# zju3dv/Diffuman4D

Measured on NVIDIA H100. Metric: unet_window_denoise_steps_per_sec, higher is better.
Workload: dtype bf16

## Files before the change

diffuman4d_b200/build.py:

```python
from __future__ import annotations

import concurrent.futures as cf
import os
import subprocess
import sys

HERE = os.path.dirname(os.path.abspath(__file__))
CSRC = os.path.join(HERE, "csrc")
OBJ = os.path.join(HERE, "_obj")
LIB = os.path.join(HERE, "libd4d.so")
SOURCES = ["tmap.cu", "gemm_wgmma.cu", "attention_wgmma.cu", "norm.cu", "elementwise.cu", "unet.cu", "d4d_api.cu"]
NVCC = os.environ.get("NVCC", "/usr/local/cuda/bin/nvcc")
FLAGS = ["-std=c++17", "-O3", "-gencode", "arch=compute_90a,code=sm_90a", "-lineinfo", "-Xcompiler", "-fPIC",
         "-diag-suppress", "177"]


def _deps_mtime() -> float:
    t = 0.0
    for root in (CSRC, os.path.join(HERE, "..", "include")):
        for f in os.listdir(root):
            if f.endswith((".h", ".cuh")):
                t = max(t, os.path.getmtime(os.path.join(root, f)))
    return t


def _compile(src: str, force: bool, hdr_t: float) -> str:
    obj = os.path.join(OBJ, src.replace(".cu", ".o"))
    s = os.path.join(CSRC, src)
    if not force and os.path.exists(obj) and os.path.getmtime(obj) >= max(os.path.getmtime(s), hdr_t):
        return obj
    cmd = [NVCC, *FLAGS, "-I", CSRC, "-c", s, "-o", obj]
    r = subprocess.run(cmd, capture_output=True, text=True)
    if r.returncode != 0:
        raise RuntimeError(f"nvcc failed for {src}:\n{r.stdout}\n{r.stderr}")
    return obj


def _link(lib: str, objs, force: bool) -> bool:
    need_link = force or not os.path.exists(lib) or any(os.path.getmtime(o) > os.path.getmtime(lib) for o in objs)
    if need_link:
        cmd = [NVCC, "-shared", "-o", lib, *objs, "-cudart", "static", "-gencode", "arch=compute_90a,code=sm_90a",
               "-Xlinker", "--exclude-libs,ALL"]
        r = subprocess.run(cmd, capture_output=True, text=True)
        if r.returncode != 0:
            raise RuntimeError(f"link failed:\n{r.stdout}\n{r.stderr}")
    return need_link


def build(force: bool = False, verbose: bool = True) -> str:
    os.makedirs(OBJ, exist_ok=True)
    hdr_t = _deps_mtime()
    with cf.ThreadPoolExecutor(max_workers=min(8, os.cpu_count() or 4)) as ex:
        objs = list(ex.map(lambda s: _compile(s, force, hdr_t), SOURCES))
    linked = _link(LIB, objs, force)
    if verbose:
        print(f"[d4d] {'built' if linked else 'up to date'}: {LIB}")
    return LIB


if __name__ == "__main__":
    build(force="--force" in sys.argv)
```

diffuman4d_b200/csrc/attention_wgmma.cu:

```cuda
#include <math.h>

#include "kernels.h"
#include "wgmma.cuh"

namespace d4d {

namespace {

constexpr int BLOCK_Q = 128;
constexpr int BLOCK_KV = 64;
constexpr int ATT_THREADS = 288;
constexpr int QBOX_BYTES = BLOCK_Q * 64 * 2;
constexpr int KVBOX_BYTES = BLOCK_KV * 64 * 2;

template <int NB>
struct AttCfg {
  static constexpr int D = 64 * NB;
  static constexpr int STAGES = NB == 3 ? 3 : 4;
  static constexpr int Q_BYTES = QBOX_BYTES * NB;
  static constexpr int STAGE_BYTES = 2 * KVBOX_BYTES * NB;
  static constexpr int SMEM_BYTES = 1024 + Q_BYTES + STAGES * STAGE_BYTES + 256;
  static constexpr int MIN_BLOCKS = NB == 1 ? 2 : 1;
};

struct AttKernelArgs {
  int seq_q, seq_kv, heads, n_kv_tiles;
  float scale_log2;
  bf16* out;
  int ld_out;
};

__device__ __forceinline__ float ex2_approx(float x) {
  float y;
  asm("ex2.approx.ftz.f32 %0, %1;" : "=f"(y) : "f"(x));
  return y;
}

template <int NB>
__global__ void __launch_bounds__(ATT_THREADS, AttCfg<NB>::MIN_BLOCKS)
attn_wgmma_kernel(const __grid_constant__ CUtensorMap tmap_q, const __grid_constant__ CUtensorMap tmap_k,
                  const __grid_constant__ CUtensorMap tmap_v, const AttKernelArgs a) {
  using C = AttCfg<NB>;
  extern __shared__ uint8_t smem_raw[];
  uint8_t* smem = reinterpret_cast<uint8_t*>((reinterpret_cast<uintptr_t>(smem_raw) + 1023) & ~uintptr_t(1023));
  uint8_t* sQ = smem;
  uint8_t* ring = smem + C::Q_BYTES;
  uint64_t* kv_full = reinterpret_cast<uint64_t*>(ring + C::STAGES * C::STAGE_BYTES);
  uint64_t* kv_empty = kv_full + C::STAGES;
  uint64_t* q_full = kv_empty + C::STAGES;

  const int warp = __shfl_sync(0xffffffffu, threadIdx.x >> 5, 0);
  const int lane = threadIdx.x & 31;
  const int q_tile = blockIdx.x;
  const int bh = blockIdx.y;
  const int b = bh / a.heads;
  const int hd = bh - b * a.heads;
  const int q_row0 = b * a.seq_q;
  const int kv_row0 = b * a.seq_kv;
  const int col0 = hd * C::D;
  const int n_tiles = a.n_kv_tiles;

  if (threadIdx.x == 0) {
    for (int i = 0; i < C::STAGES; ++i) {
      mbar_init(&kv_full[i], 1);
      mbar_init(&kv_empty[i], 2);
    }
    mbar_init(q_full, 1);
    fence_mbar_init();
  }
  __syncthreads();
  pdl_wait();
  pdl_launch_dependents();

  if (warp == 8) {
    if (lane == 0) {
      tma_prefetch_desc(&tmap_q);
      tma_prefetch_desc(&tmap_k);
      tma_prefetch_desc(&tmap_v);
      mbar_expect_tx(q_full, C::Q_BYTES);
#pragma unroll
      for (int nb = 0; nb < NB; ++nb)
        tma_load_2d(sQ + nb * QBOX_BYTES, &tmap_q, q_full, col0 + nb * 64, q_row0 + q_tile * BLOCK_Q);
      int stage = 0;
      uint32_t phase = 0;
      for (int j = 0; j < n_tiles; ++j) {
        mbar_wait(&kv_empty[stage], phase ^ 1);
        uint8_t* dst = ring + stage * C::STAGE_BYTES;
        mbar_expect_tx(&kv_full[stage], C::STAGE_BYTES);
#pragma unroll
        for (int nb = 0; nb < NB; ++nb) {
          tma_load_2d(dst + nb * KVBOX_BYTES, &tmap_k, &kv_full[stage], col0 + nb * 64, kv_row0 + j * BLOCK_KV);
          tma_load_2d(dst + (NB + nb) * KVBOX_BYTES, &tmap_v, &kv_full[stage], col0 + nb * 64, kv_row0 + j * BLOCK_KV);
        }
        if (++stage == C::STAGES) { stage = 0; phase ^= 1; }
      }
    }
    return;
  }

  const int wg = warp >> 2;
  const bool wg_leader = (threadIdx.x & 127) == 0;
  const int c_base = 2 * (lane & 3);
  const uint32_t q_addr = smem_u32(sQ) + wg * 64 * 128;
  const uint32_t ring_u32 = smem_u32(ring);

  float o[NB][32];
#pragma unroll
  for (int nb = 0; nb < NB; ++nb)
#pragma unroll
    for (int i = 0; i < 32; ++i) o[nb][i] = 0.f;
  float m_run[2] = {-INFINITY, -INFINITY};
  float l_run[2] = {0.f, 0.f};
  mbar_wait(q_full, 0);

  int stage = 0;
  uint32_t phase = 0;
  for (int j = 0; j < n_tiles; ++j) {
    mbar_wait(&kv_full[stage], phase);
    const uint32_t kv = ring_u32 + stage * C::STAGE_BYTES;
    float s[32];
    wgmma_fence();
#pragma unroll
    for (int nb = 0; nb < NB; ++nb) {
      const uint64_t qd = make_wgmma_desc(q_addr + nb * QBOX_BYTES, 16, 1024);
      const uint64_t kd = make_wgmma_desc(kv + nb * KVBOX_BYTES, 16, 1024);
#pragma unroll
      for (int k = 0; k < 4; ++k) wgmma_ss_n64(s, qd + 2 * k, kd + 2 * k, (nb | k) != 0 ? 1 : 0);
    }
    wgmma_commit();
    wgmma_wait<0>();
    wgmma_fence_regs(s);

    const int valid = a.seq_kv - j * BLOCK_KV;
    if (valid < BLOCK_KV) {
#pragma unroll
      for (int i = 0; i < 32; ++i)
        if (8 * (i >> 2) + c_base + (i & 1) >= valid) s[i] = -INFINITY;
    }
    float corr[2];
#pragma unroll
    for (int h = 0; h < 2; ++h) {
      float mx = -INFINITY;
#pragma unroll
      for (int jj = 0; jj < 8; ++jj) mx = fmaxf(mx, fmaxf(s[4 * jj + 2 * h], s[4 * jj + 2 * h + 1]));
      mx = fmaxf(mx, __shfl_xor_sync(0xffffffffu, mx, 1));
      mx = fmaxf(mx, __shfl_xor_sync(0xffffffffu, mx, 2));
      const float m_new = fmaxf(m_run[h], mx * a.scale_log2);
      corr[h] = ex2_approx(m_run[h] - m_new);
      m_run[h] = m_new;
      float sum = 0.f;
#pragma unroll
      for (int jj = 0; jj < 8; ++jj) {
#pragma unroll
        for (int e = 0; e < 2; ++e) {
          const float p = ex2_approx(fmaf(s[4 * jj + 2 * h + e], a.scale_log2, -m_new));
          s[4 * jj + 2 * h + e] = p;
          sum += p;
        }
      }
      l_run[h] = l_run[h] * corr[h] + sum;
    }
#pragma unroll
    for (int nb = 0; nb < NB; ++nb)
#pragma unroll
      for (int i = 0; i < 32; ++i) o[nb][i] *= corr[(i >> 1) & 1];

    uint32_t pf[4][4];
#pragma unroll
    for (int kk = 0; kk < 4; ++kk) {
      pf[kk][0] = pack_bf16x2(s[8 * kk + 0], s[8 * kk + 1]);
      pf[kk][1] = pack_bf16x2(s[8 * kk + 2], s[8 * kk + 3]);
      pf[kk][2] = pack_bf16x2(s[8 * kk + 4], s[8 * kk + 5]);
      pf[kk][3] = pack_bf16x2(s[8 * kk + 6], s[8 * kk + 7]);
    }
    wgmma_fence();
#pragma unroll
    for (int nb = 0; nb < NB; ++nb) {
      const uint64_t vd = make_wgmma_desc(kv + (NB + nb) * KVBOX_BYTES, KVBOX_BYTES, 1024);
#pragma unroll
      for (int kk = 0; kk < 4; ++kk) wgmma_rs_n64_bmn(o[nb], pf[kk], vd + (2048 >> 4) * kk);
    }
    wgmma_commit();
    wgmma_wait<0>();
#pragma unroll
    for (int nb = 0; nb < NB; ++nb) wgmma_fence_regs(o[nb]);
    if (wg_leader) mbar_arrive(&kv_empty[stage]);
    if (++stage == C::STAGES) { stage = 0; phase ^= 1; }
  }

  const int r_base = q_tile * BLOCK_Q + wg * 64 + (warp & 3) * 16 + (lane >> 2);
#pragma unroll
  for (int h = 0; h < 2; ++h) {
    float l = l_run[h];
    l += __shfl_xor_sync(0xffffffffu, l, 1);
    l += __shfl_xor_sync(0xffffffffu, l, 2);
    const float inv_l = 1.f / l;
    const int qrow = r_base + 8 * h;
    if (qrow >= a.seq_q) continue;
    bf16* orow = a.out + static_cast<size_t>(q_row0 + qrow) * a.ld_out + col0;
#pragma unroll
    for (int nb = 0; nb < NB; ++nb)
#pragma unroll
      for (int jj = 0; jj < 8; ++jj)
        *reinterpret_cast<uint32_t*>(orow + nb * 64 + 8 * jj + c_base) =
            pack_bf16x2(o[nb][4 * jj + 2 * h] * inv_l, o[nb][4 * jj + 2 * h + 1] * inv_l);
  }
}

template <int NB>
int launch_attn(const AttnLaunch& L, cudaStream_t stream) {
  using C = AttCfg<NB>;
  static PerDeviceOnce attr_once;
  if (int rc = ensure_dyn_smem(attn_wgmma_kernel<NB>, C::SMEM_BYTES, attr_once)) return rc;
  AttKernelArgs a;
  a.seq_q = L.d.seq;
  a.seq_kv = L.d.seq_kv > 0 ? L.d.seq_kv : L.d.seq;
  a.heads = L.d.heads;
  a.n_kv_tiles = (a.seq_kv + BLOCK_KV - 1) / BLOCK_KV;
  a.scale_log2 = L.d.scale * 1.4426950408889634f;
  a.out = L.d.out;
  a.ld_out = L.d.ld_out;
  dim3 grid(L.grid_x, L.grid_y);
  D4D_CUDA_OK(launch_pdl(attn_wgmma_kernel<NB>, grid, dim3(ATT_THREADS), C::SMEM_BYTES, stream, L.tmap_q, L.tmap_k, L.tmap_v, a));
  D4D_CUDA_OK(cudaGetLastError());
  return 0;
}

}

int attn_prepare(const AttnDesc& d, AttnLaunch* L) {
  D4D_REQUIRE(d.head_dim == 64 || d.head_dim == 128 || d.head_dim == 192,
              "attention head_dim (after padding) must be 64, 128 or 192");
  D4D_REQUIRE(d.batch > 0 && d.seq > 0 && d.heads > 0 && d.seq_kv >= 0, "empty attention problem");
  D4D_REQUIRE(d.ld_qkv % 8 == 0 && d.ld_out % 8 == 0 && d.ld_kv % 8 == 0, "leading dimensions must be multiples of 8");
  D4D_REQUIRE(d.scale > 0.f, "softmax scale must be positive");
  L->d = d;
  L->variant = d.head_dim / 64;
  const int seq_kv = d.seq_kv > 0 ? d.seq_kv : d.seq;
  const int ld_kv = d.ld_kv > 0 ? d.ld_kv : d.ld_qkv;
  const uint64_t q_tokens = static_cast<uint64_t>(d.batch) * d.seq;
  const uint64_t kv_tokens = static_cast<uint64_t>(d.batch) * seq_kv;
  const uint64_t width = static_cast<uint64_t>(d.heads) * d.head_dim;
  if (int rc = make_tmap_2d(&L->tmap_q, d.q, q_tokens, width, d.ld_qkv, 64, BLOCK_Q, 128)) return rc;
  if (int rc = make_tmap_2d(&L->tmap_k, d.k, kv_tokens, width, ld_kv, 64, BLOCK_KV, 128)) return rc;
  if (int rc = make_tmap_2d(&L->tmap_v, d.v, kv_tokens, width, ld_kv, 64, BLOCK_KV, 128)) return rc;
  L->grid_x = (d.seq + BLOCK_Q - 1) / BLOCK_Q;
  L->grid_y = d.batch * d.heads;
  D4D_REQUIRE(L->grid_y <= 65535, "batch*heads exceeds grid.y limit");
  return 0;
}

int attn_run(const AttnLaunch& L, cudaStream_t stream) {
  switch (L.variant) {
    case 1: return launch_attn<1>(L, stream);
    case 2: return launch_attn<2>(L, stream);
    case 3: return launch_attn<3>(L, stream);
  }
  set_error("attention: unsupported head_dim variant");
  return 1;
}

double attn_flops(const AttnDesc& d) {
  const double skv = d.seq_kv > 0 ? d.seq_kv : d.seq;
  return 4.0 * d.batch * d.heads * static_cast<double>(d.seq) * skv * d.head_dim;
}

}
```

diffuman4d_b200/csrc/wgmma.cuh:

```cuda
#pragma once
#include <stdint.h>

namespace d4d {

__device__ __forceinline__ void wgmma_fence() { asm volatile("wgmma.fence.sync.aligned;" ::: "memory"); }
__device__ __forceinline__ void wgmma_commit() { asm volatile("wgmma.commit_group.sync.aligned;" ::: "memory"); }
template <int N> __device__ __forceinline__ void wgmma_wait() {
  asm volatile("wgmma.wait_group.sync.aligned %0;" ::"n"(N) : "memory");
}
template <int R> __device__ __forceinline__ void wgmma_fence_regs(float (&d)[R]) {
#pragma unroll
  for (int i = 0; i < R; ++i) asm volatile("" : "+f"(d[i])::"memory");
}

__device__ __forceinline__ uint64_t make_wgmma_desc(uint32_t saddr, uint32_t lbo_bytes, uint32_t sbo_bytes) {
  uint64_t d = 0;
  d |= static_cast<uint64_t>((saddr >> 4) & 0x3FFFu);
  d |= static_cast<uint64_t>((lbo_bytes >> 4) & 0x3FFFu) << 16;
  d |= static_cast<uint64_t>((sbo_bytes >> 4) & 0x3FFFu) << 32;
  d |= 1ull << 62;
  return d;
}


__device__ __forceinline__ void wgmma_ss_n64(float (&d)[32], uint64_t a_desc, uint64_t b_desc, int scale_d) {
  asm volatile(
      "{\n\t.reg .pred p;\n\t"
      "setp.ne.b32 p, %34, 0;\n\t"
      "wgmma.mma_async.sync.aligned.m64n64k16.f32.bf16.bf16 {%0, %1, %2, %3, %4, %5, %6, %7, %8, %9, %10, %11, %12, %13, %14, %15, %16, %17, %18, %19, %20, %21, %22, %23, %24, %25, %26, %27, %28, %29, %30, %31}, %32, %33, p, 1, 1, 0, 0;\n\t}\n"
      : "+f"(d[0]), "+f"(d[1]), "+f"(d[2]), "+f"(d[3]), "+f"(d[4]), "+f"(d[5]), "+f"(d[6]), "+f"(d[7]), "+f"(d[8]), "+f"(d[9]), "+f"(d[10]), "+f"(d[11]), "+f"(d[12]), "+f"(d[13]), "+f"(d[14]), "+f"(d[15]), "+f"(d[16]), "+f"(d[17]), "+f"(d[18]), "+f"(d[19]), "+f"(d[20]), "+f"(d[21]), "+f"(d[22]), "+f"(d[23]), "+f"(d[24]), "+f"(d[25]), "+f"(d[26]), "+f"(d[27]), "+f"(d[28]), "+f"(d[29]), "+f"(d[30]), "+f"(d[31])
      : "l"(a_desc), "l"(b_desc), "r"(scale_d));
}

__device__ __forceinline__ void wgmma_ss_n128(float (&d)[64], uint64_t a_desc, uint64_t b_desc, int scale_d) {
  asm volatile(
      "{\n\t.reg .pred p;\n\t"
      "setp.ne.b32 p, %66, 0;\n\t"
      "wgmma.mma_async.sync.aligned.m64n128k16.f32.bf16.bf16 {%0, %1, %2, %3, %4, %5, %6, %7, %8, %9, %10, %11, %12, %13, %14, %15, %16, %17, %18, %19, %20, %21, %22, %23, %24, %25, %26, %27, %28, %29, %30, %31, %32, %33, %34, %35, %36, %37, %38, %39, %40, %41, %42, %43, %44, %45, %46, %47, %48, %49, %50, %51, %52, %53, %54, %55, %56, %57, %58, %59, %60, %61, %62, %63}, %64, %65, p, 1, 1, 0, 0;\n\t}\n"
      : "+f"(d[0]), "+f"(d[1]), "+f"(d[2]), "+f"(d[3]), "+f"(d[4]), "+f"(d[5]), "+f"(d[6]), "+f"(d[7]), "+f"(d[8]), "+f"(d[9]), "+f"(d[10]), "+f"(d[11]), "+f"(d[12]), "+f"(d[13]), "+f"(d[14]), "+f"(d[15]), "+f"(d[16]), "+f"(d[17]), "+f"(d[18]), "+f"(d[19]), "+f"(d[20]), "+f"(d[21]), "+f"(d[22]), "+f"(d[23]), "+f"(d[24]), "+f"(d[25]), "+f"(d[26]), "+f"(d[27]), "+f"(d[28]), "+f"(d[29]), "+f"(d[30]), "+f"(d[31]), "+f"(d[32]), "+f"(d[33]), "+f"(d[34]), "+f"(d[35]), "+f"(d[36]), "+f"(d[37]), "+f"(d[38]), "+f"(d[39]), "+f"(d[40]), "+f"(d[41]), "+f"(d[42]), "+f"(d[43]), "+f"(d[44]), "+f"(d[45]), "+f"(d[46]), "+f"(d[47]), "+f"(d[48]), "+f"(d[49]), "+f"(d[50]), "+f"(d[51]), "+f"(d[52]), "+f"(d[53]), "+f"(d[54]), "+f"(d[55]), "+f"(d[56]), "+f"(d[57]), "+f"(d[58]), "+f"(d[59]), "+f"(d[60]), "+f"(d[61]), "+f"(d[62]), "+f"(d[63])
      : "l"(a_desc), "l"(b_desc), "r"(scale_d));
}

__device__ __forceinline__ void wgmma_ss_n160(float (&d)[80], uint64_t a_desc, uint64_t b_desc, int scale_d) {
  asm volatile(
      "{\n\t.reg .pred p;\n\t"
      "setp.ne.b32 p, %82, 0;\n\t"
      "wgmma.mma_async.sync.aligned.m64n160k16.f32.bf16.bf16 {%0, %1, %2, %3, %4, %5, %6, %7, %8, %9, %10, %11, %12, %13, %14, %15, %16, %17, %18, %19, %20, %21, %22, %23, %24, %25, %26, %27, %28, %29, %30, %31, %32, %33, %34, %35, %36, %37, %38, %39, %40, %41, %42, %43, %44, %45, %46, %47, %48, %49, %50, %51, %52, %53, %54, %55, %56, %57, %58, %59, %60, %61, %62, %63, %64, %65, %66, %67, %68, %69, %70, %71, %72, %73, %74, %75, %76, %77, %78, %79}, %80, %81, p, 1, 1, 0, 0;\n\t}\n"
      : "+f"(d[0]), "+f"(d[1]), "+f"(d[2]), "+f"(d[3]), "+f"(d[4]), "+f"(d[5]), "+f"(d[6]), "+f"(d[7]), "+f"(d[8]), "+f"(d[9]), "+f"(d[10]), "+f"(d[11]), "+f"(d[12]), "+f"(d[13]), "+f"(d[14]), "+f"(d[15]), "+f"(d[16]), "+f"(d[17]), "+f"(d[18]), "+f"(d[19]), "+f"(d[20]), "+f"(d[21]), "+f"(d[22]), "+f"(d[23]), "+f"(d[24]), "+f"(d[25]), "+f"(d[26]), "+f"(d[27]), "+f"(d[28]), "+f"(d[29]), "+f"(d[30]), "+f"(d[31]), "+f"(d[32]), "+f"(d[33]), "+f"(d[34]), "+f"(d[35]), "+f"(d[36]), "+f"(d[37]), "+f"(d[38]), "+f"(d[39]), "+f"(d[40]), "+f"(d[41]), "+f"(d[42]), "+f"(d[43]), "+f"(d[44]), "+f"(d[45]), "+f"(d[46]), "+f"(d[47]), "+f"(d[48]), "+f"(d[49]), "+f"(d[50]), "+f"(d[51]), "+f"(d[52]), "+f"(d[53]), "+f"(d[54]), "+f"(d[55]), "+f"(d[56]), "+f"(d[57]), "+f"(d[58]), "+f"(d[59]), "+f"(d[60]), "+f"(d[61]), "+f"(d[62]), "+f"(d[63]), "+f"(d[64]), "+f"(d[65]), "+f"(d[66]), "+f"(d[67]), "+f"(d[68]), "+f"(d[69]), "+f"(d[70]), "+f"(d[71]), "+f"(d[72]), "+f"(d[73]), "+f"(d[74]), "+f"(d[75]), "+f"(d[76]), "+f"(d[77]), "+f"(d[78]), "+f"(d[79])
      : "l"(a_desc), "l"(b_desc), "r"(scale_d));
}

__device__ __forceinline__ void wgmma_ss_n192(float (&d)[96], uint64_t a_desc, uint64_t b_desc, int scale_d) {
  asm volatile(
      "{\n\t.reg .pred p;\n\t"
      "setp.ne.b32 p, %98, 0;\n\t"
      "wgmma.mma_async.sync.aligned.m64n192k16.f32.bf16.bf16 {%0, %1, %2, %3, %4, %5, %6, %7, %8, %9, %10, %11, %12, %13, %14, %15, %16, %17, %18, %19, %20, %21, %22, %23, %24, %25, %26, %27, %28, %29, %30, %31, %32, %33, %34, %35, %36, %37, %38, %39, %40, %41, %42, %43, %44, %45, %46, %47, %48, %49, %50, %51, %52, %53, %54, %55, %56, %57, %58, %59, %60, %61, %62, %63, %64, %65, %66, %67, %68, %69, %70, %71, %72, %73, %74, %75, %76, %77, %78, %79, %80, %81, %82, %83, %84, %85, %86, %87, %88, %89, %90, %91, %92, %93, %94, %95}, %96, %97, p, 1, 1, 0, 0;\n\t}\n"
      : "+f"(d[0]), "+f"(d[1]), "+f"(d[2]), "+f"(d[3]), "+f"(d[4]), "+f"(d[5]), "+f"(d[6]), "+f"(d[7]), "+f"(d[8]), "+f"(d[9]), "+f"(d[10]), "+f"(d[11]), "+f"(d[12]), "+f"(d[13]), "+f"(d[14]), "+f"(d[15]), "+f"(d[16]), "+f"(d[17]), "+f"(d[18]), "+f"(d[19]), "+f"(d[20]), "+f"(d[21]), "+f"(d[22]), "+f"(d[23]), "+f"(d[24]), "+f"(d[25]), "+f"(d[26]), "+f"(d[27]), "+f"(d[28]), "+f"(d[29]), "+f"(d[30]), "+f"(d[31]), "+f"(d[32]), "+f"(d[33]), "+f"(d[34]), "+f"(d[35]), "+f"(d[36]), "+f"(d[37]), "+f"(d[38]), "+f"(d[39]), "+f"(d[40]), "+f"(d[41]), "+f"(d[42]), "+f"(d[43]), "+f"(d[44]), "+f"(d[45]), "+f"(d[46]), "+f"(d[47]), "+f"(d[48]), "+f"(d[49]), "+f"(d[50]), "+f"(d[51]), "+f"(d[52]), "+f"(d[53]), "+f"(d[54]), "+f"(d[55]), "+f"(d[56]), "+f"(d[57]), "+f"(d[58]), "+f"(d[59]), "+f"(d[60]), "+f"(d[61]), "+f"(d[62]), "+f"(d[63]), "+f"(d[64]), "+f"(d[65]), "+f"(d[66]), "+f"(d[67]), "+f"(d[68]), "+f"(d[69]), "+f"(d[70]), "+f"(d[71]), "+f"(d[72]), "+f"(d[73]), "+f"(d[74]), "+f"(d[75]), "+f"(d[76]), "+f"(d[77]), "+f"(d[78]), "+f"(d[79]), "+f"(d[80]), "+f"(d[81]), "+f"(d[82]), "+f"(d[83]), "+f"(d[84]), "+f"(d[85]), "+f"(d[86]), "+f"(d[87]), "+f"(d[88]), "+f"(d[89]), "+f"(d[90]), "+f"(d[91]), "+f"(d[92]), "+f"(d[93]), "+f"(d[94]), "+f"(d[95])
      : "l"(a_desc), "l"(b_desc), "r"(scale_d));
}

__device__ __forceinline__ void wgmma_ss_n256(float (&d)[128], uint64_t a_desc, uint64_t b_desc, int scale_d) {
  asm volatile(
      "{\n\t.reg .pred p;\n\t"
      "setp.ne.b32 p, %130, 0;\n\t"
      "wgmma.mma_async.sync.aligned.m64n256k16.f32.bf16.bf16 {%0, %1, %2, %3, %4, %5, %6, %7, %8, %9, %10, %11, %12, %13, %14, %15, %16, %17, %18, %19, %20, %21, %22, %23, %24, %25, %26, %27, %28, %29, %30, %31, %32, %33, %34, %35, %36, %37, %38, %39, %40, %41, %42, %43, %44, %45, %46, %47, %48, %49, %50, %51, %52, %53, %54, %55, %56, %57, %58, %59, %60, %61, %62, %63, %64, %65, %66, %67, %68, %69, %70, %71, %72, %73, %74, %75, %76, %77, %78, %79, %80, %81, %82, %83, %84, %85, %86, %87, %88, %89, %90, %91, %92, %93, %94, %95, %96, %97, %98, %99, %100, %101, %102, %103, %104, %105, %106, %107, %108, %109, %110, %111, %112, %113, %114, %115, %116, %117, %118, %119, %120, %121, %122, %123, %124, %125, %126, %127}, %128, %129, p, 1, 1, 0, 0;\n\t}\n"
      : "+f"(d[0]), "+f"(d[1]), "+f"(d[2]), "+f"(d[3]), "+f"(d[4]), "+f"(d[5]), "+f"(d[6]), "+f"(d[7]), "+f"(d[8]), "+f"(d[9]), "+f"(d[10]), "+f"(d[11]), "+f"(d[12]), "+f"(d[13]), "+f"(d[14]), "+f"(d[15]), "+f"(d[16]), "+f"(d[17]), "+f"(d[18]), "+f"(d[19]), "+f"(d[20]), "+f"(d[21]), "+f"(d[22]), "+f"(d[23]), "+f"(d[24]), "+f"(d[25]), "+f"(d[26]), "+f"(d[27]), "+f"(d[28]), "+f"(d[29]), "+f"(d[30]), "+f"(d[31]), "+f"(d[32]), "+f"(d[33]), "+f"(d[34]), "+f"(d[35]), "+f"(d[36]), "+f"(d[37]), "+f"(d[38]), "+f"(d[39]), "+f"(d[40]), "+f"(d[41]), "+f"(d[42]), "+f"(d[43]), "+f"(d[44]), "+f"(d[45]), "+f"(d[46]), "+f"(d[47]), "+f"(d[48]), "+f"(d[49]), "+f"(d[50]), "+f"(d[51]), "+f"(d[52]), "+f"(d[53]), "+f"(d[54]), "+f"(d[55]), "+f"(d[56]), "+f"(d[57]), "+f"(d[58]), "+f"(d[59]), "+f"(d[60]), "+f"(d[61]), "+f"(d[62]), "+f"(d[63]), "+f"(d[64]), "+f"(d[65]), "+f"(d[66]), "+f"(d[67]), "+f"(d[68]), "+f"(d[69]), "+f"(d[70]), "+f"(d[71]), "+f"(d[72]), "+f"(d[73]), "+f"(d[74]), "+f"(d[75]), "+f"(d[76]), "+f"(d[77]), "+f"(d[78]), "+f"(d[79]), "+f"(d[80]), "+f"(d[81]), "+f"(d[82]), "+f"(d[83]), "+f"(d[84]), "+f"(d[85]), "+f"(d[86]), "+f"(d[87]), "+f"(d[88]), "+f"(d[89]), "+f"(d[90]), "+f"(d[91]), "+f"(d[92]), "+f"(d[93]), "+f"(d[94]), "+f"(d[95]), "+f"(d[96]), "+f"(d[97]), "+f"(d[98]), "+f"(d[99]), "+f"(d[100]), "+f"(d[101]), "+f"(d[102]), "+f"(d[103]), "+f"(d[104]), "+f"(d[105]), "+f"(d[106]), "+f"(d[107]), "+f"(d[108]), "+f"(d[109]), "+f"(d[110]), "+f"(d[111]), "+f"(d[112]), "+f"(d[113]), "+f"(d[114]), "+f"(d[115]), "+f"(d[116]), "+f"(d[117]), "+f"(d[118]), "+f"(d[119]), "+f"(d[120]), "+f"(d[121]), "+f"(d[122]), "+f"(d[123]), "+f"(d[124]), "+f"(d[125]), "+f"(d[126]), "+f"(d[127])
      : "l"(a_desc), "l"(b_desc), "r"(scale_d));
}

__device__ __forceinline__ void wgmma_rs_n64_bmn(float (&d)[32], const uint32_t (&a)[4], uint64_t b_desc) {
  asm volatile(
      "wgmma.mma_async.sync.aligned.m64n64k16.f32.bf16.bf16 {%0, %1, %2, %3, %4, %5, %6, %7, %8, %9, %10, %11, %12, %13, %14, %15, %16, %17, %18, %19, %20, %21, %22, %23, %24, %25, %26, %27, %28, %29, %30, %31}, {%32, %33, %34, %35}, %36, 1, 1, 1, 1;\n"
      : "+f"(d[0]), "+f"(d[1]), "+f"(d[2]), "+f"(d[3]), "+f"(d[4]), "+f"(d[5]), "+f"(d[6]), "+f"(d[7]), "+f"(d[8]), "+f"(d[9]), "+f"(d[10]), "+f"(d[11]), "+f"(d[12]), "+f"(d[13]), "+f"(d[14]), "+f"(d[15]), "+f"(d[16]), "+f"(d[17]), "+f"(d[18]), "+f"(d[19]), "+f"(d[20]), "+f"(d[21]), "+f"(d[22]), "+f"(d[23]), "+f"(d[24]), "+f"(d[25]), "+f"(d[26]), "+f"(d[27]), "+f"(d[28]), "+f"(d[29]), "+f"(d[30]), "+f"(d[31])
      : "r"(a[0]), "r"(a[1]), "r"(a[2]), "r"(a[3]), "l"(b_desc));
}

}
```

Measured before the change: 14.58.

## Pipeline attention QK and PV wgmma with warp specialization and per-variant KV tiles

Restructures the attention kernel so the next tile's QK^T wgmma is issued together with the current tile's PV wgmma, overlapping softmax with tensor-core work. It adds a full producer warpgroup with setmaxnreg register rebalancing between producer and consumers. It also sizes the KV block per head-dim variant (128 for D=64, smaller for larger heads) and fills the stage count up to the shared-memory limit. The build now fails if ptxas reports serialized wgmma; the risks are higher register pressure and only one block per SM.

```diff
diff --git a/diffuman4d_b200/build.py b/diffuman4d_b200/build.py
--- a/diffuman4d_b200/build.py
+++ b/diffuman4d_b200/build.py
@@ -33,6 +33,10 @@
     r = subprocess.run(cmd, capture_output=True, text=True)
     if r.returncode != 0:
         raise RuntimeError(f"nvcc failed for {src}:\n{r.stdout}\n{r.stderr}")
+    serialized = [ln for ln in (r.stdout + r.stderr).splitlines() if "wgmma.mma_async instructions are serialized" in ln]
+    if serialized:
+        os.remove(obj)
+        raise RuntimeError(f"ptxas serialized the wgmma of {src}:\n" + "\n".join(serialized))
     return obj
 
 
diff --git a/diffuman4d_b200/csrc/attention_wgmma.cu b/diffuman4d_b200/csrc/attention_wgmma.cu
--- a/diffuman4d_b200/csrc/attention_wgmma.cu
+++ b/diffuman4d_b200/csrc/attention_wgmma.cu
@@ -8,19 +8,19 @@
 namespace {
 
 constexpr int BLOCK_Q = 128;
-constexpr int BLOCK_KV = 64;
-constexpr int ATT_THREADS = 288;
+constexpr int ATT_THREADS = 384;
 constexpr int QBOX_BYTES = BLOCK_Q * 64 * 2;
-constexpr int KVBOX_BYTES = BLOCK_KV * 64 * 2;
+constexpr int ATT_SMEM_MAX = 227 * 1024;
 
 template <int NB>
 struct AttCfg {
   static constexpr int D = 64 * NB;
-  static constexpr int STAGES = NB == 3 ? 3 : 4;
+  static constexpr int BLOCK_KV = NB == 1 ? 128 : 64 / (NB - 1);
+  static constexpr int KVBOX_BYTES = BLOCK_KV * 64 * 2;
   static constexpr int Q_BYTES = QBOX_BYTES * NB;
   static constexpr int STAGE_BYTES = 2 * KVBOX_BYTES * NB;
+  static constexpr int STAGES = (ATT_SMEM_MAX - 1024 - 256 - Q_BYTES) / STAGE_BYTES;
   static constexpr int SMEM_BYTES = 1024 + Q_BYTES + STAGES * STAGE_BYTES + 256;
-  static constexpr int MIN_BLOCKS = NB == 1 ? 2 : 1;
 };
 
 struct AttKernelArgs {
@@ -36,11 +36,55 @@
   return y;
 }
 
+template <int BKV, bool kMask>
+__device__ __forceinline__ void softmax_tile(float (&s)[BKV / 2], int valid, int c_base, float scale_log2,
+                                             float (&m_run)[2], float (&l_run)[2], float (&corr)[2]) {
+  if (kMask && valid < BKV) {
+#pragma unroll
+    for (int i = 0; i < BKV / 2; ++i)
+      if (8 * (i >> 2) + c_base + (i & 1) >= valid) s[i] = -INFINITY;
+  }
+#pragma unroll
+  for (int h = 0; h < 2; ++h) {
+    float mx = -INFINITY;
+#pragma unroll
+    for (int jj = 0; jj < BKV / 8; ++jj) mx = fmaxf(mx, fmaxf(s[4 * jj + 2 * h], s[4 * jj + 2 * h + 1]));
+    mx = fmaxf(mx, __shfl_xor_sync(0xffffffffu, mx, 1));
+    mx = fmaxf(mx, __shfl_xor_sync(0xffffffffu, mx, 2));
+    const float m_new = fmaxf(m_run[h], mx * scale_log2);
+    corr[h] = ex2_approx(m_run[h] - m_new);
+    m_run[h] = m_new;
+    float sum = 0.f;
+#pragma unroll
+    for (int jj = 0; jj < BKV / 8; ++jj) {
+#pragma unroll
+      for (int e = 0; e < 2; ++e) {
+        const float p = ex2_approx(fmaf(s[4 * jj + 2 * h + e], scale_log2, -m_new));
+        s[4 * jj + 2 * h + e] = p;
+        sum += p;
+      }
+    }
+    l_run[h] = l_run[h] * corr[h] + sum;
+  }
+}
+
+template <int BKV>
+__device__ __forceinline__ void pack_p(const float (&s)[BKV / 2], uint32_t (&pf)[BKV / 16][4]) {
+#pragma unroll
+  for (int kk = 0; kk < BKV / 16; ++kk) {
+    pf[kk][0] = pack_bf16x2(s[8 * kk + 0], s[8 * kk + 1]);
+    pf[kk][1] = pack_bf16x2(s[8 * kk + 2], s[8 * kk + 3]);
+    pf[kk][2] = pack_bf16x2(s[8 * kk + 4], s[8 * kk + 5]);
+    pf[kk][3] = pack_bf16x2(s[8 * kk + 6], s[8 * kk + 7]);
+  }
+}
+
 template <int NB>
-__global__ void __launch_bounds__(ATT_THREADS, AttCfg<NB>::MIN_BLOCKS)
+__global__ void __launch_bounds__(ATT_THREADS, 1)
 attn_wgmma_kernel(const __grid_constant__ CUtensorMap tmap_q, const __grid_constant__ CUtensorMap tmap_k,
                   const __grid_constant__ CUtensorMap tmap_v, const AttKernelArgs a) {
   using C = AttCfg<NB>;
+  constexpr int BKV = C::BLOCK_KV;
   extern __shared__ uint8_t smem_raw[];
   uint8_t* smem = reinterpret_cast<uint8_t*>((reinterpret_cast<uintptr_t>(smem_raw) + 1023) & ~uintptr_t(1023));
   uint8_t* sQ = smem;
@@ -72,8 +116,9 @@
   pdl_wait();
   pdl_launch_dependents();
 
-  if (warp == 8) {
-    if (lane == 0) {
+  if (warp < 4) {
+    setmaxnreg_dec<40>();
+    if (threadIdx.x == 0) {
       tma_prefetch_desc(&tmap_q);
       tma_prefetch_desc(&tmap_k);
       tma_prefetch_desc(&tmap_v);
@@ -84,13 +129,13 @@
       int stage = 0;
       uint32_t phase = 0;
       for (int j = 0; j < n_tiles; ++j) {
-        mbar_wait(&kv_empty[stage], phase ^ 1);
+        mbar_wait_nocall(&kv_empty[stage], phase ^ 1);
         uint8_t* dst = ring + stage * C::STAGE_BYTES;
         mbar_expect_tx(&kv_full[stage], C::STAGE_BYTES);
 #pragma unroll
         for (int nb = 0; nb < NB; ++nb) {
-          tma_load_2d(dst + nb * KVBOX_BYTES, &tmap_k, &kv_full[stage], col0 + nb * 64, kv_row0 + j * BLOCK_KV);
-          tma_load_2d(dst + (NB + nb) * KVBOX_BYTES, &tmap_v, &kv_full[stage], col0 + nb * 64, kv_row0 + j * BLOCK_KV);
+          tma_load_2d(dst + nb * C::KVBOX_BYTES, &tmap_k, &kv_full[stage], col0 + nb * 64, kv_row0 + j * BKV);
+          tma_load_2d(dst + (NB + nb) * C::KVBOX_BYTES, &tmap_v, &kv_full[stage], col0 + nb * 64, kv_row0 + j * BKV);
         }
         if (++stage == C::STAGES) { stage = 0; phase ^= 1; }
       }
@@ -98,11 +143,42 @@
     return;
   }
 
-  const int wg = warp >> 2;
+  setmaxnreg_inc<232>();
+  const int wg = (warp >> 2) - 1;
   const bool wg_leader = (threadIdx.x & 127) == 0;
   const int c_base = 2 * (lane & 3);
+  const int r_wg = wg * 64 + (warp & 3) * 16 + (lane >> 2);
+  const uint32_t ring_u32 = smem_u32(ring);
+
   const uint32_t q_addr = smem_u32(sQ) + wg * 64 * 128;
-  const uint32_t ring_u32 = smem_u32(ring);
+  mbar_wait_nocall(q_full, 0);
+
+  const auto issue_s = [&](float (&s)[BKV / 2], int stg) {
+    const uint32_t kv = ring_u32 + stg * C::STAGE_BYTES;
+#pragma unroll
+    for (int nb = 0; nb < NB; ++nb) {
+      const uint64_t qd = make_wgmma_desc(q_addr + nb * QBOX_BYTES, 16, 1024);
+      const uint64_t kd = make_wgmma_desc(kv + nb * C::KVBOX_BYTES, 16, 1024);
+#pragma unroll
+      for (int k = 0; k < 4; ++k) {
+        if constexpr (BKV == 128) wgmma_ss_n128(s, qd + 2 * k, kd + 2 * k, (nb | k) != 0 ? 1 : 0);
+        else if constexpr (BKV == 64) wgmma_ss_n64(s, qd + 2 * k, kd + 2 * k, (nb | k) != 0 ? 1 : 0);
+        else wgmma_ss_n32(s, qd + 2 * k, kd + 2 * k, (nb | k) != 0 ? 1 : 0);
+      }
+    }
+    wgmma_commit();
+  };
+
+  const auto issue_pv = [&](float (&o)[NB][32], const uint32_t (&pf)[BKV / 16][4], int stg) {
+    const uint32_t kv = ring_u32 + stg * C::STAGE_BYTES;
+#pragma unroll
+    for (int nb = 0; nb < NB; ++nb) {
+      const uint64_t vd = make_wgmma_desc(kv + (NB + nb) * C::KVBOX_BYTES, C::KVBOX_BYTES, 1024);
+#pragma unroll
+      for (int kk = 0; kk < BKV / 16; ++kk) wgmma_rs_n64_bmn(o[nb], pf[kk], vd + (2048 >> 4) * kk);
+    }
+    wgmma_commit();
+  };
 
   float o[NB][32];
 #pragma unroll
@@ -111,91 +187,57 @@
     for (int i = 0; i < 32; ++i) o[nb][i] = 0.f;
   float m_run[2] = {-INFINITY, -INFINITY};
   float l_run[2] = {0.f, 0.f};
-  mbar_wait(q_full, 0);
+  float corr[2];
+  float s[BKV / 2];
+  uint32_t pf[BKV / 16][4];
+
+  mbar_wait_nocall(&kv_full[0], 0);
+  wgmma_fence();
+  issue_s(s, 0);
+  wgmma_wait<0>();
+  wgmma_fence_regs(s);
+  softmax_tile<BKV, true>(s, a.seq_kv, c_base, a.scale_log2, m_run, l_run, corr);
+  pack_p<BKV>(s, pf);
 
   int stage = 0;
   uint32_t phase = 0;
-  for (int j = 0; j < n_tiles; ++j) {
-    mbar_wait(&kv_full[stage], phase);
-    const uint32_t kv = ring_u32 + stage * C::STAGE_BYTES;
-    float s[32];
+  for (int j = 0; j + 1 < n_tiles; ++j) {
+    int next = stage + 1;
+    uint32_t next_phase = phase;
+    if (next == C::STAGES) { next = 0; next_phase ^= 1; }
+    mbar_wait_nocall(&kv_full[next], next_phase);
     wgmma_fence();
+    issue_s(s, next);
+    issue_pv(o, pf, stage);
+    wgmma_wait<1>();
+    wgmma_fence_regs(s);
+    if (j + 2 < n_tiles) softmax_tile<BKV, false>(s, BKV, c_base, a.scale_log2, m_run, l_run, corr);
+    else softmax_tile<BKV, true>(s, a.seq_kv - (j + 1) * BKV, c_base, a.scale_log2, m_run, l_run, corr);
+    wgmma_wait<0>();
 #pragma unroll
     for (int nb = 0; nb < NB; ++nb) {
-      const uint64_t qd = make_wgmma_desc(q_addr + nb * QBOX_BYTES, 16, 1024);
-      const uint64_t kd = make_wgmma_desc(kv + nb * KVBOX_BYTES, 16, 1024);
-#pragma unroll
-      for (int k = 0; k < 4; ++k) wgmma_ss_n64(s, qd + 2 * k, kd + 2 * k, (nb | k) != 0 ? 1 : 0);
-    }
-    wgmma_commit();
-    wgmma_wait<0>();
-    wgmma_fence_regs(s);
-
-    const int valid = a.seq_kv - j * BLOCK_KV;
-    if (valid < BLOCK_KV) {
-#pragma unroll
-      for (int i = 0; i < 32; ++i)
-        if (8 * (i >> 2) + c_base + (i & 1) >= valid) s[i] = -INFINITY;
-    }
-    float corr[2];
-#pragma unroll
-    for (int h = 0; h < 2; ++h) {
-      float mx = -INFINITY;
-#pragma unroll
-      for (int jj = 0; jj < 8; ++jj) mx = fmaxf(mx, fmaxf(s[4 * jj + 2 * h], s[4 * jj + 2 * h + 1]));
-      mx = fmaxf(mx, __shfl_xor_sync(0xffffffffu, mx, 1));
-      mx = fmaxf(mx, __shfl_xor_sync(0xffffffffu, mx, 2));
-      const float m_new = fmaxf(m_run[h], mx * a.scale_log2);
-      corr[h] = ex2_approx(m_run[h] - m_new);
-      m_run[h] = m_new;
-      float sum = 0.f;
-#pragma unroll
-      for (int jj = 0; jj < 8; ++jj) {
-#pragma unroll
-        for (int e = 0; e < 2; ++e) {
-          const float p = ex2_approx(fmaf(s[4 * jj + 2 * h + e], a.scale_log2, -m_new));
-          s[4 * jj + 2 * h + e] = p;
-          sum += p;
-        }
-      }
-      l_run[h] = l_run[h] * corr[h] + sum;
-    }
-#pragma unroll
-    for (int nb = 0; nb < NB; ++nb)
+      wgmma_fence_regs(o[nb]);
 #pragma unroll
       for (int i = 0; i < 32; ++i) o[nb][i] *= corr[(i >> 1) & 1];
-
-    uint32_t pf[4][4];
-#pragma unroll
-    for (int kk = 0; kk < 4; ++kk) {
-      pf[kk][0] = pack_bf16x2(s[8 * kk + 0], s[8 * kk + 1]);
-      pf[kk][1] = pack_bf16x2(s[8 * kk + 2], s[8 * kk + 3]);
-      pf[kk][2] = pack_bf16x2(s[8 * kk + 4], s[8 * kk + 5]);
-      pf[kk][3] = pack_bf16x2(s[8 * kk + 6], s[8 * kk + 7]);
-    }
-    wgmma_fence();
-#pragma unroll
-    for (int nb = 0; nb < NB; ++nb) {
-      const uint64_t vd = make_wgmma_desc(kv + (NB + nb) * KVBOX_BYTES, KVBOX_BYTES, 1024);
-#pragma unroll
-      for (int kk = 0; kk < 4; ++kk) wgmma_rs_n64_bmn(o[nb], pf[kk], vd + (2048 >> 4) * kk);
-    }
-    wgmma_commit();
-    wgmma_wait<0>();
-#pragma unroll
-    for (int nb = 0; nb < NB; ++nb) wgmma_fence_regs(o[nb]);
+    }
+    pack_p<BKV>(s, pf);
     if (wg_leader) mbar_arrive(&kv_empty[stage]);
-    if (++stage == C::STAGES) { stage = 0; phase ^= 1; }
-  }
-
-  const int r_base = q_tile * BLOCK_Q + wg * 64 + (warp & 3) * 16 + (lane >> 2);
+    stage = next;
+    phase = next_phase;
+  }
+  wgmma_fence();
+  issue_pv(o, pf, stage);
+  wgmma_wait<0>();
+#pragma unroll
+  for (int nb = 0; nb < NB; ++nb) wgmma_fence_regs(o[nb]);
+
 #pragma unroll
   for (int h = 0; h < 2; ++h) {
     float l = l_run[h];
     l += __shfl_xor_sync(0xffffffffu, l, 1);
     l += __shfl_xor_sync(0xffffffffu, l, 2);
     const float inv_l = 1.f / l;
-    const int qrow = r_base + 8 * h;
+    const int qrow = q_tile * BLOCK_Q + r_wg + 8 * h;
     if (qrow >= a.seq_q) continue;
     bf16* orow = a.out + static_cast<size_t>(q_row0 + qrow) * a.ld_out + col0;
 #pragma unroll
@@ -216,7 +258,7 @@
   a.seq_q = L.d.seq;
   a.seq_kv = L.d.seq_kv > 0 ? L.d.seq_kv : L.d.seq;
   a.heads = L.d.heads;
-  a.n_kv_tiles = (a.seq_kv + BLOCK_KV - 1) / BLOCK_KV;
+  a.n_kv_tiles = (a.seq_kv + C::BLOCK_KV - 1) / C::BLOCK_KV;
   a.scale_log2 = L.d.scale * 1.4426950408889634f;
   a.out = L.d.out;
   a.ld_out = L.d.ld_out;
@@ -224,6 +266,14 @@
   D4D_CUDA_OK(launch_pdl(attn_wgmma_kernel<NB>, grid, dim3(ATT_THREADS), C::SMEM_BYTES, stream, L.tmap_q, L.tmap_k, L.tmap_v, a));
   D4D_CUDA_OK(cudaGetLastError());
   return 0;
+}
+
+int attn_block_kv(int variant) {
+  switch (variant) {
+    case 1: return AttCfg<1>::BLOCK_KV;
+    case 2: return AttCfg<2>::BLOCK_KV;
+    default: return AttCfg<3>::BLOCK_KV;
+  }
 }
 
 }
@@ -242,8 +292,9 @@
   const uint64_t kv_tokens = static_cast<uint64_t>(d.batch) * seq_kv;
   const uint64_t width = static_cast<uint64_t>(d.heads) * d.head_dim;
   if (int rc = make_tmap_2d(&L->tmap_q, d.q, q_tokens, width, d.ld_qkv, 64, BLOCK_Q, 128)) return rc;
-  if (int rc = make_tmap_2d(&L->tmap_k, d.k, kv_tokens, width, ld_kv, 64, BLOCK_KV, 128)) return rc;
-  if (int rc = make_tmap_2d(&L->tmap_v, d.v, kv_tokens, width, ld_kv, 64, BLOCK_KV, 128)) return rc;
+  const uint32_t block_kv = attn_block_kv(L->variant);
+  if (int rc = make_tmap_2d(&L->tmap_k, d.k, kv_tokens, width, ld_kv, 64, block_kv, 128)) return rc;
+  if (int rc = make_tmap_2d(&L->tmap_v, d.v, kv_tokens, width, ld_kv, 64, block_kv, 128)) return rc;
   L->grid_x = (d.seq + BLOCK_Q - 1) / BLOCK_Q;
   L->grid_y = d.batch * d.heads;
   D4D_REQUIRE(L->grid_y <= 65535, "batch*heads exceeds grid.y limit");
diff --git a/diffuman4d_b200/csrc/wgmma.cuh b/diffuman4d_b200/csrc/wgmma.cuh
--- a/diffuman4d_b200/csrc/wgmma.cuh
+++ b/diffuman4d_b200/csrc/wgmma.cuh
@@ -22,6 +22,15 @@
   return d;
 }
 
+
+__device__ __forceinline__ void wgmma_ss_n32(float (&d)[16], uint64_t a_desc, uint64_t b_desc, int scale_d) {
+  asm volatile(
+      "{\n\t.reg .pred p;\n\t"
+      "setp.ne.b32 p, %18, 0;\n\t"
+      "wgmma.mma_async.sync.aligned.m64n32k16.f32.bf16.bf16 {%0, %1, %2, %3, %4, %5, %6, %7, %8, %9, %10, %11, %12, %13, %14, %15}, %16, %17, p, 1, 1, 0, 0;\n\t}\n"
+      : "+f"(d[0]), "+f"(d[1]), "+f"(d[2]), "+f"(d[3]), "+f"(d[4]), "+f"(d[5]), "+f"(d[6]), "+f"(d[7]), "+f"(d[8]), "+f"(d[9]), "+f"(d[10]), "+f"(d[11]), "+f"(d[12]), "+f"(d[13]), "+f"(d[14]), "+f"(d[15])
+      : "l"(a_desc), "l"(b_desc), "r"(scale_d));
+}
 
 __device__ __forceinline__ void wgmma_ss_n64(float (&d)[32], uint64_t a_desc, uint64_t b_desc, int scale_d) {
   asm volatile(
```

Measured after the change: 14.60, median of 6. Within noise of the previous version (+0.1%).
